# Chthi/Ofighters

Measured on AMD Instinct MI355X. Metric: arena-steps/sec (env.step+obs+policy fwd) at 4096 arenas, 1/2/4/8 MI355X, higher is better.
Workload: dtype f32; 1 GPU; 4096 arenas x 8 ships per GPU, random-bot actions + step + 2D obs rasterise (u8 maps) + bi-head policy forward for 8 ship(s)/arena, trunk shared per arena (BASELINE configs[3]); arenas_per_gpu=4096, ships=8, laser_cap=512, episode_ticks=200, parallelism=arena-sharded x1, RCCL all-reduce of episodic scores only, laser_overflow=0, last_episode_score_sum=70993, last_episode_arenas=4096

## Files before the change

ofighters_amd/csrc/ofx_head.hip:

```cpp
#include "ofx_head.h"
#include "ofx_lowp.h"
#include "ofx_diag.h"
#include <stdlib.h>


typedef float f32x4 __attribute__((ext_vector_type(4)));
typedef float f32x2 __attribute__((ext_vector_type(2)));
#define HD_PS 400
constexpr int HC4_ZERO = 800;
constexpr int HC4_COL = 816, HC4_CPITCH = 416;
constexpr int HC4_STRIDE = HC4_COL + 2 * HC4_CPITCH + 16;
__device__ __forceinline__ int hc4_at(int ln, int t) { return ln < 2 ? ln * 400 + t : HC4_COL + (ln - 2) * HC4_CPITCH + t; }
__device__ __forceinline__ int hc4_pad(int k) { return k < 16 ? HC4_ZERO + k : k < 32 ? HC4_COL + 400 + k - 16 : HC4_COL + HC4_CPITCH + 400 + k - 32; }

__device__ __forceinline__ void hc4_zero_block(const HeadParams2 &p, int tid, int threads) {
  if (blockIdx.x == 0)
    for (int e = tid; e < HC4_STRIDE; e += threads) p.c4[(size_t)p.S * HC4_STRIDE + e] = 0.f;
}

__device__ __forceinline__ float hd_max_raw(float x, float floor) {
  float pinf;
  asm("s_mov_b32 %0, 0x7f800000" : "=s"(pinf));
  return __builtin_amdgcn_fmed3f(x, floor, pinf);
}
// ... 125 lines not shown
    if (t >= 0 && t < 200) {
      int fa, fb, ta, tb; float wf, wt;
      hf_taps(f, 100, fa, fb, wf, p.legacy);
      hf_taps(t, 100, ta, tb, wt, p.legacy);
      const int ba = fa < 2 ? fa : fa - 96, bb = fb < 2 ? fb : fb - 96;
      const float *src = isc ? u2cb : u2rb;
      const float a = src[(ba * 100 + ta) * 4 + ci], bq = src[(ba * 100 + tb) * 4 + ci];
      const float d = src[(bb * 100 + ta) * 4 + ci], g = src[(bb * 100 + tb) * 4 + ci];
      if (!isc) {
        const float top = a + (bq - a) * wt, bot = d + (g - d) * wt;
        v = top + (bot - top) * wf;
      } else {
        const float top = a + (d - a) * wf, bot = bq + (g - bq) * wf;
        v = top + (bot - top) * wt;
      }
    }
    (isc ? U2c : U2r)[(b * 4 + ci) * 202 + t + 1] = v;
  }
  __syncthreads();

  for (int e = tid; e < 4 * 200 * 8; e += HF_THREADS) {
    const int co = e % 8, t = (e / 8) % 200, ln = e / 1600, isc = ln >> 1;
    const int f = (ln & 1) ? 199 : 0;
    float acc = p.b3[co];
#pragma unroll
    for (int d0 = 0; d0 < 3; d0++) {
      const int u = f + d0 - 1;
      if (u < 0 || u > 199) continue;
      const int ub = u < 2 ? u : u - 196;
#pragma unroll
      for (int d1 = 0; d1 < 3; d1++)
#pragma unroll
        for (int ci = 0; ci < 4; ci++) {
          const int dy = isc ? d1 : d0, dx = isc ? d0 : d1;
          const float uv = (isc ? U2c : U2r)[(ub * 4 + ci) * 202 + t + d1];
          acc += p.w3raw[((dy * 3 + dx) * 4 + ci) * 8 + co] * uv;
        }
    }
    u3l[(ln * 200 + t) * 8 + co] = fmaxf(acc, 0.f);
  }
  __syncthreads();
  if (tid < 32) {
    const int co = tid & 7, c = tid >> 3;
    const int rl = (c & 1) ? 1 : 0, x = (c & 2) ? 199 : 0;
    const int cl = (c & 2) ? 3 : 2, y = (c & 1) ? 199 : 0;
    u3l[(cl * 200 + y) * 8 + co] = u3l[(rl * 200 + x) * 8 + co];
  }
  __syncthreads();
  for (int e = tid; e < 4 * 200 * 9; e += HF_THREADS) {
    const int tp = e % 9, cell = e / 9;
    float acc = 0.f;
    for (int ci = 0; ci < 8; ci++) acc = fmaf(p.w4raw[tp * 8 + ci], u3l[cell * 8 + ci], acc);
    p.vfr[(size_t)s * 7200 + e] = acc;
  }

  for (int e = tid; e < 4 * 400; e += HF_THREADS) {
    const int ln = e / 400, t = e - ln * 400, isc = ln >> 1, side = ln & 1;
    float acc = 0.f;
    if (!isc || (t > 0 && t < 399)) {
      const int d0 = side ? 2 : 0;
#pragma unroll
      for (int d1 = 0; d1 < 3; d1++)
#pragma unroll
        for (int ci = 0; ci < 8; ci++) {
          const int tap = isc ? d1 * 3 + d0 : d0 * 3 + d1;
          acc += p.w4raw[tap * 8 + ci] * hf_up(u3l + ln * 1600 + ci, 8, 200, t + d1 - 1, p.legacy);
        }
      if (!isc && (t == 0 || t == 399)) {
        const int cl = t ? 3 : 2, dx = t ? 2 : 0;
        for (int dy = 0; dy < 3; dy++) {
          if (dy == d0) continue;
          const int yy = (side ? 399 : 0) + dy - 1;
          if (yy < 0 || yy > 399) continue;
          for (int ci = 0; ci < 8; ci++) acc += p.w4raw[(dy * 3 + dx) * 8 + ci] * hf_up(u3l + cl * 1600 + ci, 8, 200, yy, p.legacy);
        }
      }
    }
    p.c4[(size_t)s * HC4_STRIDE + hc4_at(ln, t)] = acc;
  }
  if (tid < 64) p.c4[(size_t)s * HC4_STRIDE + hc4_pad(tid)] = 0.f;
}

constexpr int HG_THREADS = 256;
constexpr int HG_L1 = 0;
constexpr int HG_U3 = 0;
constexpr int HG_RB = 6400;
constexpr int HG_CB = HG_RB + 4 * 102 * 4;
constexpr int HG_TOTAL = HG_CB + 4 * 102 * 4;
static_assert(2 * 52 * 52 <= 6400, "l1p fits under u3l");

template <int CIN, int COUT>
__device__ __forceinline__ void hg_corner_w(const float *w, int yc, int xc, int co, float (&wr)[4 * CIN]) {
  const int dy0 = yc == 0 ? 1 : 0, dx0 = xc == 0 ? 1 : 0;
#pragma unroll
  for (int t = 0; t < 4; t++)
#pragma unroll
    for (int ci = 0; ci < CIN; ci++) wr[t * CIN + ci] = w[(((dy0 + (t >> 1)) * 3 + dx0 + (t & 1)) * CIN + ci) * COUT + co];
}
template <int CIN, class G>
__device__ __forceinline__ float hg_corner(G get, int n, int yc, int xc, const float (&wr)[4 * CIN], float bias, int legacy) {
  float acc = bias;
  const int dy0 = yc == 0 ? 1 : 0, dx0 = xc == 0 ? 1 : 0;
#pragma unroll
  for (int a2 = 0; a2 < 2; a2++) {
    int ya, yb; float wy;
    hf_taps(yc + dy0 + a2 - 1, n, ya, yb, wy, legacy);
#pragma unroll
    for (int b2 = 0; b2 < 2; b2++) {
      int xa, xb; float wx;
      hf_taps(xc + dx0 + b2 - 1, n, xa, xb, wx, legacy);
#pragma unroll
      for (int ci = 0; ci < CIN; ci++) {
        const float a = get(ya, xa, ci), b = get(ya, xb, ci), d = get(yb, xa, ci), g = get(yb, xb, ci);
        const float top = a + (b - a) * wx, bot = d + (g - d) * wx;
        acc += wr[(a2 * 2 + b2) * CIN + ci] * (top + (bot - top) * wy);
      }
    }
  }
  return fmaxf(acc, 0.f);
}

constexpr int HG_NB = 6 * 52 + 46 * 6, HG_NE = 2 * HG_NB, HG_PER = (HG_NE + HG_THREADS - 1) / HG_THREADS;
struct alignas(16) HgStage { unsigned v[HG_PER * HG_THREADS]; };
constexpr HgStage hg_make_stage() {
  HgStage t{};
  for (int e0 = 0; e0 < HG_PER * HG_THREADS; e0++) {
    const int e = e0 < HG_NE ? e0 : HG_NE - 1;
    const int ci = e / HG_NB, k = e - ci * HG_NB;
    int r = 0, c = 0;
    if (k < 6 * 52) { const int rr = k / 52; r = rr < 3 ? rr : rr + 46; c = k - rr * 52; }
    else { const int k2 = k - 6 * 52, cc = k2 % 6; r = 3 + k2 / 6; c = cc < 3 ? cc : cc + 46; }
    const int rs = r - 1 < 0 ? 0 : r - 1 > 49 ? 49 : r - 1, cs = c - 1 < 0 ? 0 : c - 1 > 49 ? 49 : c - 1;
    t.v[e0] = (unsigned)((ci * 52 + r) * 52 + c) | (unsigned)((ci * 50 + rs) * 50 + cs) << 16;
  }
  return t;
}
__constant__ HgStage kHgStage = hg_make_stage();

__global__ __launch_bounds__(HG_THREADS) void k_head_frames(HeadParams2 p) {
  __shared__ __align__(16) float sm[HG_TOTAL];
  __shared__ float efr_s[192], w4s[72];
  const int s = hd_ship(p, (int)((blockIdx.x & ~7u) | ((blockIdx.x + (blockIdx.x >> 3)) & 7u)));
  const int tid = threadIdx.x, lane = tid & 63;
  hc4_zero_block(p, tid, HG_THREADS);
  if (s < 0) return;
  const int wv = __builtin_amdgcn_readfirstlane(tid >> 6);
  const int n16 = lane & 15, kq = lane >> 4;
  float *l1p = sm + HG_L1, *u2rb = sm + HG_RB, *u2cb = sm + HG_CB, *u3l = sm + HG_U3;

  constexpr int NE = HG_NE, PER = HG_PER;
  unsigned at[PER];
#pragma unroll
  for (int u = 0; u < PER; u++) at[u] = kHgStage.v[u * HG_THREADS + tid];
  const float efr_v = p.efr[min(tid, 191)], w4_v = p.w4raw[min(tid, 71)];
  float bw2[5];
#pragma unroll
  for (int jj = 0; jj < 5; jj++) bw2[jj] = p.w2fr[(wv * 20 + 4 * jj + kq) * 16 + n16];
  float bw3[9];
#pragma unroll
  for (int jj = 0; jj < 9; jj++) bw3[jj] = p.w3fr[(wv * 36 + 4 * jj + kq) * 16 + n16];
  const float b2v = p.b2[n16 & 3], b3v = p.b3[n16 & 7];
  float wc2[8], wc3[16];
  if (wv == 0) {
    hg_corner_w<2, 4>(p.w2raw, (lane >> 5) ? 99 : 0, ((lane >> 4) & 1) ? 99 : 0, lane & 3, wc2);
    hg_corner_w<4, 8>(p.w3raw, ((lane >> 3) & 1) ? 199 : 0, ((lane >> 3) & 2) ? 199 : 0, lane & 7, wc3);
  }
  {
    float v[PER];
    const float *src = p.up1 + (size_t)s * 5000;
#pragma unroll
    for (int u = 0; u < PER; u++) v[u] = src[at[u] >> 16];
#pragma unroll
    for (int u = 0; u < PER; u++)
      if (u * HG_THREADS + tid < NE) l1p[at[u] & 0xFFFFu] = v[u];
  }
  if (tid < 192) efr_s[tid] = efr_v;
  if (tid < 72) w4s[tid] = w4_v;
  __syncthreads();

#pragma unroll 1
  for (int m = 0; m < 4; m++) {
    const int v = wv;
    const int pp = min(16 * m + n16, 49);
    const int i = v == 0 ? 0 : v == 1 ? 49 : pp, j = v == 2 ? 0 : v == 3 ? 49 : pp;
    const float bias = b2v;
    f32x4 d = {bias, bias, bias, bias};
#pragma unroll
    for (int jj = 0; jj < 5; jj++) {
      const int tap = min(2 * jj + (kq >> 1), 8);
      const float a = l1p[((kq & 1) * 52 + i + tap / 3) * 52 + j + tap % 3];
      d = __builtin_amdgcn_mfma_f32_16x16x4f32(a, bw2[jj], d, 0, 0, 0);
    }
    const int co = n16 & 3, pa = n16 >> 3, pb = (n16 >> 2) & 1;
#pragma unroll
    for (int r = 0; r < 4; r++) {
      const int q = 16 * m + 4 * kq + r;
      if (q >= 50) continue;
      const float val = fmaxf(d[r], 0.f);
      if (v < 2) {
        u2rb[((2 * v + pa) * 102 + 2 * q + pb + 1) * 4 + co] = val;
      } else {
        u2cb[((2 * (v - 2) + pb) * 102 + 2 * q + pa + 1) * 4 + co] = val;
      }
    }
  }
  __syncthreads();
  if (tid < 64) {
    const int co = tid & 3, cx = (tid >> 2) & 1, cy = (tid >> 3) & 1, bx = (tid >> 4) & 1, by = tid >> 5;
    const int y = by ? 98 + cy : cy, x = bx ? 98 + cx : cx;
    const int rb = by ? 2 + cy : cy, cb = bx ? 2 + cx : cx;
    const bool fy = y == 0 || y == 99, fx = x == 0 || x == 99;
    float val;
    if (fy && fx) {
      auto get = [&](int yy, int xx, int ci) { return l1p[(ci * 52 + yy + 1) * 52 + xx + 1]; };
      val = hg_corner<2>(get, 50, y, x, wc2, b2v, p.legacy);
    } else if (fx) {
      val = u2cb[(cb * 102 + y + 1) * 4 + co];
    } else {
      val = u2rb[(rb * 102 + x + 1) * 4 + co];
    }
    if (fy && fx) { u2rb[(rb * 102 + x + 1) * 4 + co] = val; u2cb[(cb * 102 + y + 1) * 4 + co] = val; }
    else if (fx) u2rb[(rb * 102 + x + 1) * 4 + co] = val;
    else u2cb[(cb * 102 + y + 1) * 4 + co] = val;
  }
  __syncthreads();
  if (tid < 128) {
    const int co = tid & 3, b = (tid >> 2) & 3, hi = (tid >> 4) & 1, isc = tid >> 5;
    if (isc < 2) {
      float *ln = (isc ? u2cb : u2rb) + b * 102 * 4;
      ln[(hi ? 101 : 0) * 4 + co] = ln[(hi ? 100 : 1) * 4 + co];
    }
  }
  {
    const float *src = (wv < 2 ? u2rb : u2cb) + ((wv & 1) ? 3 : 0) * 408 + 4;
    float *dst = p.u2fr + (size_t)s * 1600 + wv * 400;
#pragma unroll
    for (int k = 0; k < 7; k++) {
      const int r = lane + 64 * k;
      if (r < 400) dst[r] = src[r];
    }
  }
  __syncthreads();

#pragma unroll 1
  for (int m = 0; m < 7; m++) {
    const int v = wv;
    const int qq = min(16 * m + n16, 99);
    const float *band = (v < 2 ? u2rb : u2cb);
    const int b0 = (v & 1) ? 2 : 0;
    const float bias = b3v;
    f32x4 d = {bias, bias, bias, bias};
#pragma unroll
    for (int jj = 0; jj < 9; jj++) {
      const int ty = jj / 3, tx = jj % 3;
      const int tf = v < 2 ? ty : tx, ta = v < 2 ? tx : ty;
      const int bsel = (v & 1) ? b0 + min(tf, 1) : b0 + max(tf - 1, 0);
      const float a = band[(bsel * 102 + qq + ta) * 4 + kq];
      d = __builtin_amdgcn_mfma_f32_16x16x4f32(a, bw3[jj], d, 0, 0, 0);
    }
    const int co = n16 & 7, par = n16 >> 3;
#pragma unroll
    for (int r = 0; r < 4; r++) {
      const int q = 16 * m + 4 * kq + r;
      if (q < 100) u3l[(v * 200 + 2 * q + par) * 8 + co] = fmaxf(d[r], 0.f);
    }
  }
  __syncthreads();
  if (tid < 32) {
    const int co = tid & 7, c = tid >> 3;
    const int y = (c & 1) ? 199 : 0, x = (c & 2) ? 199 : 0;
    auto get = [&](int yy, int xx, int ci) {
      return u2rb[((yy < 50 ? yy : yy - 96) * 102 + xx + 1) * 4 + ci];
    };
    const float val = hg_corner<4>(get, 100, y, x, wc3, b3v, p.legacy);
    u3l[(((c & 1) ? 1 : 0) * 200 + x) * 8 + co] = val;
    u3l[(((c & 2) ? 3 : 2) * 200 + y) * 8 + co] = val;
  }
  __syncthreads();
  if (tid < 252) {
    const int tp = tid % 9, c0 = tid / 9;
    float wt[8];
#pragma unroll
    for (int ci = 0; ci < 8; ci++) wt[ci] = w4s[tp * 8 + ci];
    float *dst = p.vfr + (size_t)s * 7200 + tid;
    for (int cell = c0; cell < 4 * 200; cell += 28) {
      const f32x4 ua = *reinterpret_cast<const f32x4 *>(u3l + cell * 8), ub = *reinterpret_cast<const f32x4 *>(u3l + cell * 8 + 4);
      float acc = 0.f;
#pragma unroll
      for (int ci = 0; ci < 4; ci++) acc = fmaf(wt[ci], ua[ci], acc);
#pragma unroll
      for (int ci = 0; ci < 4; ci++) acc = fmaf(wt[4 + ci], ub[ci], acc);
      dst[(cell - c0) * 9] = acc;
    }
  }

  {
    const int ln = wv, isc = ln >> 1, side = ln & 1;
    const float *L = u3l + ln * 1600;
    float E[24];
#pragma unroll
    for (int i = 0; i < 24; i++) E[i] = efr_s[(ln * 2 + (lane & 1)) * 24 + i];
    float *dst = p.c4 + (size_t)s * HC4_STRIDE + hc4_at(ln, 0);
#pragma unroll 1
    for (int k = 0; k < 7; k++) {
      const int t = lane + 64 * k, jq = t >> 1;
      float acc = 0.f;
#pragma unroll
      for (int o = 0; o < 3; o++) {
        const float *Lp = L + min(max(jq + o - 1, 0), 199) * 8;
        const f32x4 la = *reinterpret_cast<const f32x4 *>(Lp), lb = *reinterpret_cast<const f32x4 *>(Lp + 4);
#pragma unroll
        for (int ci = 0; ci < 4; ci++) acc += E[o * 8 + ci] * la[ci];
#pragma unroll
        for (int ci = 0; ci < 4; ci++) acc += E[o * 8 + 4 + ci] * lb[ci];
      }
      if (isc && (t == 0 || t == 399)) acc = 0.f;
      if (!isc && (t == 0 || t == 399)) {
        const int cs = t ? 1 : 0;
        const int yq = side ? 199 : 0, a = side ? 1 : 0;
        const float *E2 = efr_s + ((2 + cs) * 2 + a) * 24;
        const float *L2 = u3l + (2 + cs) * 1600;
        for (int o = 0; o < 3; o++) {
          const float *Lp = L2 + min(max(yq + o - 1, 0), 199) * 8;
          for (int ci = 0; ci < 8; ci++) acc += E2[o * 8 + ci] * Lp[ci];
        }
        const int tap = (side ? 2 : 0) * 3 + (cs ? 2 : 0);
        const float *Lc = L + (t ? 199 : 0) * 8;
        for (int ci = 0; ci < 8; ci++) acc -= w4s[tap * 8 + ci] * Lc[ci];
      }
      if (t < 400) dst[t] = acc;
    }
  }
  if (tid < 64) p.c4[(size_t)s * HC4_STRIDE + hc4_pad(tid)] = 0.f;
}

constexpr int HS_GPR = 13;
constexpr int HS_NTILES = 325;
constexpr int HS_NS = 42;
constexpr int HS_NR3 = 16, HS_P3 = 106;
constexpr int HS_PL3 = HS_NR3 * HS_P3 + 4;
constexpr int HS_NV = 9;
constexpr int HS_NR2 = 16, HS_P2 = 56;
constexpr int HS_PL2 = (HS_NR2 + 2) * HS_P2;
static_assert(HS_PL2 % 32 == 16, "uprelu2 plane stride");
constexpr int HS_TABP = 16 * HS_GPR;
static_assert(HS_TABP == 4 * 52, "table period in tiles");
static_assert(4 * (HS_NV * HS_PL3 + 4 * HS_PL2 + HS_TABP + 400) <= 80 * 1024, "two workgroups per CU");
struct alignas(16) HsPick { signed char v[HS_NS][4]; };
constexpr int hs_pairs_done_c(int s) { return s + 2 + ((s + 2) >> 2) < 50 ? s + 2 + ((s + 2) >> 2) : 50; }
constexpr HsPick hs_make_pick() {
  HsPick t{};
  for (int st = 0; st < HS_NS; st++)
    for (int cw = 0; cw < 4; cw++) {
      const int lo = 2 * hs_pairs_done_c(st), hi = 2 * hs_pairs_done_c(st + 1);
      const int at = lo + ((cw - lo) & 3);
      t.v[st][cw] = (signed char)(at < hi ? at >> 1 : -1);
    }
  return t;
}
__constant__ HsPick kHsPick = hs_make_pick();

__device__ __forceinline__ int hs_tiles_done(int s) {
  return s < 0 ? 0 : min(HS_NTILES, 8 * (s + 1) + ((s + 1) >> 3));
}

typedef const volatile __attribute__((address_space(3))) f32x2 hs_lds_v2;

__device__ __forceinline__ void hs_u2_store(float *u2r, int ch, int row, int col, float v) {
  const int slot = (row + 1) & (HS_NR2 - 1);
  float *q = &u2r[ch * HS_PL2 + slot * HS_P2 + col];
  q[0] = v;
  if (slot < 2) q[HS_NR2 * HS_P2] = v;
}

constexpr bool HS_NZ[2][3][3] = {{{1, 1, 0}, {1, 1, 0}, {0, 1, 1}}, {{1, 1, 0}, {0, 1, 1}, {0, 1, 1}}};
constexpr float HS_CH[2][3][3] = {{{0.75f, 0.25f, 0.f}, {0.25f, 0.75f, 0.f}, {0.f, 0.75f, 0.25f}},
                                  {{0.25f, 0.75f, 0.f}, {0.f, 0.75f, 0.25f}, {0.f, 0.25f, 0.75f}}};
constexpr float HS_CL[2][3][3] = {{{0.5f, 0.5f, 0.f}, {0.f, 1.f, 0.f}, {0.f, 0.5f, 0.5f}},
                                  {{0.f, 1.f, 0.f}, {0.f, 0.5f, 0.5f}, {0.f, 0.f, 1.f}}};
static_assert(HS_CH[0][0][0] == HS_CH[0][2][1] && HS_CH[0][0][1] == HS_CH[0][2][2] && HS_CH[1][0][0] == HS_CH[1][2][1] &&
              HS_CH[1][0][1] == HS_CH[1][2][2] && HS_CL[0][0][0] == HS_CL[0][2][1] && HS_CL[0][0][1] == HS_CL[0][2][2] &&
              HS_CL[1][0][0] == HS_CL[1][2][1] && HS_CL[1][0][1] == HS_CL[1][2][2], "the stencil shares the sums of the outer taps");
constexpr int HS_NKT = 7;
constexpr int HS_KT[HS_NKT][2] = {{0, 0}, {0, 1}, {1, 0}, {1, 1}, {1, 2}, {2, 1}, {2, 2}};
__device__ __forceinline__ f32x2 hs_fma2(float c, f32x2 v, f32x2 z) { return __builtin_elementwise_fma((f32x2){c, c}, v, z); }

// ... 533 lines not shown
```

ofighters_amd/csrc/ofx_policy.hip:

```cpp
#include <string.h>

#include "ofx_internal.h"
#include "ofx_blob.h"
#include "ofx_trunk.h"
#include "ofx_head.h"

typedef float f32x16 __attribute__((ext_vector_type(16)));
typedef float f32x4 __attribute__((ext_vector_type(4)));


extern "C" int ofx_policy_layout(const ofx_handle *h, ofx_policy_desc *desc) {
  (void)h;
  if (!desc) { ofx_set_error("ofx_policy_layout: null desc"); return OFX_ERR_INVALID; }
  memset(desc, 0, sizeof(*desc));
  desc->n_tensors = policy_layout(desc->offset, desc->count);
  desc->n_floats = desc->offset[desc->n_tensors];
  return OFX_OK;
}

struct PrepLayout {
  int tw[4], tb[4];
  int uw[3], ub[3];
  int w3mf;
  int w2mf;
// ... 334 lines not shown
    }
    if (u == NB0) {
#pragma unroll
      for (int i = NB0 + NB1; i < NU; i++) a[i] = *reinterpret_cast<const f32x4 *>(ap + 4 * i);
    }
    if ((u & 1) == 0) b4[u >> 1] = *reinterpret_cast<const f32x4 *>(bl + (u >> 1) * 2 * 32 * 4);
    acc = __builtin_amdgcn_mfma_f32_32x32x2f32(kh ? a[u][1] : a[u][0], b4[u >> 1][(2 * u) & 3], acc, 0, 0, 0);
    acc = __builtin_amdgcn_mfma_f32_32x32x2f32(kh ? a[u][3] : a[u][2], b4[u >> 1][(2 * u + 1) & 3], acc, 0, 0, 0);
  }
  if (cv) {
    const float bv = bias ? bias[c] : 0.f;
#pragma unroll
    for (int i = 0; i < 16; i++) {
      const int row = m0 + (i & 3) + 8 * (i >> 2) + 4 * kh;
      if (row < M) {
        float v = acc[i] + bv;
        if (relu) v = fmaxf(v, 0.f);
        C[(size_t)(live ? live[1 + row] : row) * ldc + c] = v;
      }
    }
  }
}

constexpr int kSplitKc = 200;
__global__ __launch_bounds__(256) void k_gemm_f32_splitk(const float *A, int lda, const float *B, int ldb, float *P,
                                                         int M, int N, int tiles_n, int groups_m) {
  constexpr int Kc = kSplitKc, KG = Kc / 4, STEPS = Kc / 8;
  __shared__ __align__(16) float bs[KG * 32 * 4];
  const int tid = threadIdx.x, lane = tid & 63, wv = __builtin_amdgcn_readfirstlane(tid >> 6);
  const int nt = blockIdx.x % tiles_n, rest = blockIdx.x / tiles_n, mg = rest % groups_m, chunk = rest / groups_m;
  const int m0 = (mg * 4 + wv) * 32, n0 = nt * 32;
  const int r = m0 + (lane & 31), c = n0 + (lane & 31), kh = lane >> 5;
  const bool rv = r < M, cv = c < N;
  {
    const float *bp = B + (size_t)chunk * Kc * ldb + (n0 + (tid & 31) < N ? n0 + (tid & 31) : 0);
    f32x4 w[(KG + 7) / 8];
#pragma unroll
    for (int i = 0; i < (KG + 7) / 8; i++) {
      const int g = min((tid >> 5) + 8 * i, KG - 1);
#pragma unroll
      for (int j = 0; j < 4; j++) w[i][j] = bp[(size_t)(4 * g + j) * ldb];
    }
#pragma unroll
    for (int i = 0; i < (KG + 7) / 8; i++) {
      const int g = (tid >> 5) + 8 * i;
      if (g < KG) *reinterpret_cast<f32x4 *>(bs + (g * 32 + (tid & 31)) * 4) = w[i];
    }
  }
  const float *ap = A + (size_t)(rv ? r : 0) * lda + (size_t)chunk * Kc + 4 * kh;
  constexpr int NB0 = 9, NB1 = 8;
  f32x4 a[STEPS];
#pragma unroll
  for (int i = 0; i < NB0; i++) a[i] = *reinterpret_cast<const f32x4 *>(ap + 8 * i);
  __syncthreads();
  if (m0 >= M) return;
  f32x16 acc;
#pragma unroll
  for (int i = 0; i < 16; i++) acc[i] = 0.f;
  const float *bl = bs + (kh * 32 + (lane & 31)) * 4;
#pragma unroll
  for (int s = 0; s < STEPS; s++) {
    if (s == 0) {
#pragma unroll
      for (int i = NB0; i < NB0 + NB1; i++) a[i] = *reinterpret_cast<const f32x4 *>(ap + 8 * i);
    }
    if (s == NB0) {
#pragma unroll
      for (int i = NB0 + NB1; i < STEPS; i++) a[i] = *reinterpret_cast<const f32x4 *>(ap + 8 * i);
    }
    const f32x4 b4 = *reinterpret_cast<const f32x4 *>(bl + s * 2 * 32 * 4);
#pragma unroll
    for (int j = 0; j < 4; j++) acc = __builtin_amdgcn_mfma_f32_32x32x2f32(a[s][j], b4[j], acc, 0, 0, 0);
  }
  if (cv) {
    float *out = P + (size_t)chunk * M * N;
#pragma unroll
    for (int i = 0; i < 16; i++) {
      const int row = m0 + (i & 3) + 8 * (i >> 2) + 4 * kh;
      if (row < M) out[(size_t)row * N + c] = acc[i];
    }
  }
}

struct HeadParams {
  int N, M;
  ofx_state st;
  const float *g1;
  int g1_chunks;
  const float *k1, *b1, *k2, *b2, *k3, *b3;
  const int32_t *live;
  const uint8_t *mask;
  const float *vec8;
  float *d1;
  float *act;
  int32_t *iaction;
};

__global__ __launch_bounds__(256) void k_head_dense(HeadParams p) {
  __shared__ float sd1[4][100];
  __shared__ float sd2[4][50];
  const int lane = threadIdx.x & 63, wv = threadIdx.x >> 6;
  const int item = blockIdx.x * 4 + wv, n_items = p.live ? p.live[0] : p.N * p.M;
  if ((int)blockIdx.x * 4 >= n_items) return;
  const bool on = item < n_items;
  const int s = on ? (p.live ? p.live[1 + item] : item) : 0;
  const int a = s / p.M;
  float vec[8];
  if (on) {
    if (p.vec8) {
#pragma unroll
      for (int k = 0; k < 8; k++) vec[k] = p.vec8[(size_t)s * 8 + k];
    } else {
      vec[0] = (float)p.st.reward[s]; vec[1] = 1.f;
      vec[2] = (float)p.st.ship_px[s]; vec[3] = (float)p.st.ship_py[s];
      vec[4] = (float)PS; vec[5] = (float)PS;
      vec[6] = (float)p.st.ship_x[s]; vec[7] = (float)p.st.ship_y[s];
    }
    for (int o = lane; o < 100; o += 64) {
      float acc = 0.f;
#pragma unroll
      for (int k = 0; k < 8; k++) acc += vec[k] * p.k1[k * 100 + o];
      float g = 0.f;
      for (int ch = 0; ch < p.g1_chunks; ch++) g += p.g1[((size_t)ch * p.N + a) * 100 + o];
      acc += g;
      acc += p.b1[o];
      acc = fmaxf(acc, 0.f);
      sd1[wv][o] = acc;
      p.d1[(size_t)s * 100 + o] = acc;
    }
  }
  __syncthreads();
  if (on && lane < 50) {
    float acc = 0.f;
    for (int k = 0; k < 100; k++) acc += sd1[wv][k] * p.k2[k * 50 + lane];
    sd2[wv][lane] = fmaxf(acc + p.b2[lane], 0.f);
  }
  __syncthreads();
  if (on && lane < 2) {
    float acc = 0.f;
    for (int k = 0; k < 50; k++) acc += sd2[wv][k] * p.k3[k * 2 + lane];
    acc += p.b3[lane];
    if (p.act) p.act[(size_t)s * 2 + lane] = acc;
    const float other = __shfl_xor(acc, 1);
    if (lane == 0 && p.iaction) p.iaction[s] = other > acc ? 1 : 0;
  }
}

__device__ inline float unordered_f32(unsigned o) {
  return __uint_as_float((o & 0x80000000u) ? (o & 0x7FFFFFFFu) : ~o);
}

__global__ void k_policy_finish(int S, const uint8_t *mask, const unsigned long long *best, int32_t *ipointer,
                                float *ptr_max) {
  const int s = blockIdx.x * blockDim.x + threadIdx.x;
  if (s >= S || (mask && !mask[s])) return;
  const bool none = best[s] == 0ull;
  const unsigned k = none ? 0u : ~(unsigned)(best[s] & 0xFFFFFFFFull);
  ipointer[2 * s] = (int)(k % PS);
  ipointer[2 * s + 1] = (int)(k / PS);
  if (ptr_max) ptr_max[s] = none ? __builtin_nanf("") : unordered_f32((unsigned)(best[s] >> 32));
}

__global__ void k_policy_actions(int S, const ofx_state st, const int32_t *iaction, const int32_t *ipointer,
                                 const uint8_t *mask, ofx_action *out) {
  const int s = blockIdx.x * blockDim.x + threadIdx.x;
  if (s >= S || (mask && !mask[s])) return;
  ofx_action a;
  a.valid = st.alive[s] ? 1 : 0;
  a.shoot = iaction[s] == 0;
  a.thrust = iaction[s] == 1;
  a.px = ipointer[2 * s];
  a.py = ipointer[2 * s + 1];
  a._pad = 0;
  out[s] = a;
}

struct PolicyWs {
  float *p1, *p2, *p3, *p4, *g1, *d1, *u0, *up1, *u2fr, *vfr, *c4;
  unsigned long long *best;
  int32_t *iaction, *ipointer, *live;
};

static size_t al(size_t b) { return (b + 255) & ~(size_t)255; }
constexpr int kDense1Chunks = 25;

static int policy_workspace(ofx_handle *h, PolicyWs *ws, size_t N, size_t S) {
  size_t f2, f3, f4;
  ofx_head_frame_bytes(S, &f2, &f3, &f4);
  const size_t sz[] = {ofx_trunk_fused(h, N) ? 0 : al(4ull * N * 8 * 200 * 200), al(4ull * N * 8 * 100 * 100), al(4ull * N * 8 * 50 * 50),
                       al(4ull * N * 5000),          al(4ull * N * 100 * kDense1Chunks), al(4ull * S * 100),
                       al(4ull * S * 625),           al(4ull * S * 2 * 50 * 50),   al(f2), al(f3), al(f4),
                       al(8ull * S),                 al(4ull * S),                 al(8ull * S),
                       al(4ull * (S + 1))};
  size_t total = 0;
  for (size_t b : sz) total += b;
  int rc = ofx_ensure_scratch(h, total);
  if (rc) return rc;
  char *base = (char *)h->scratch;
  void **dst[] = {(void **)&ws->p1,   (void **)&ws->p2,   (void **)&ws->p3,      (void **)&ws->p4,      (void **)&ws->g1,
                  (void **)&ws->d1,   (void **)&ws->u0,   (void **)&ws->up1,     (void **)&ws->u2fr,    (void **)&ws->vfr,
                  (void **)&ws->c4,   (void **)&ws->best, (void **)&ws->iaction, (void **)&ws->ipointer,
                  (void **)&ws->live};
  for (size_t i = 0; i < sizeof(sz) / sizeof(sz[0]); i++) { *dst[i] = base; base += sz[i]; }
  return OFX_OK;
}

int ofx_launch_gemm(ofx_handle *h, const float *A, int lda, const float *B, int ldb, const float *bias, float *C, int ldc,
                    int M, int N, int K, int relu, const int32_t *live) {
  const int tiles_m = (M + 31) / 32, tiles_n = (N + 31) / 32, tiles = tiles_m * tiles_n;
  if (K == 100 && lda % 4 == 0 && ((uintptr_t)A & 15) == 0)
    hipLaunchKernelGGL(k_gemm_f32_k100, dim3((unsigned)(((tiles_m + 3) / 4) * tiles_n)), dim3(256), 0, h->stream, A, lda, B, ldb,
                       bias, C, ldc, M, N, relu, live, tiles_n);
  else
    hipLaunchKernelGGL(k_gemm_f32, dim3((tiles + 3) / 4), dim3(256), 0, h->stream, A, lda, B, ldb, bias, C, ldc, M, N, K,
                       relu, live);
  OFX_HIP(hipGetLastError());
  return OFX_OK;
}

static int policy_prepare(ofx_handle *h, const float *weights, float **slot) {
  const PrepLayout L = prep_layout();
  if (!*slot) {
    OFX_HIP(hipMalloc((void **)slot, sizeof(float) * L.total));
    OFX_HIP(hipMemsetAsync(*slot, 0, sizeof(float) * L.total, h->stream));
  }
  int32_t off[64], cnt[64];
  policy_layout(off, cnt);
  PrepParams pp;
  pp.w = weights; pp.prep = *slot;
  for (int i = 0; i < 4; i++) {
    pp.src_k[i] = off[ofx_t_trunk(i)]; pp.src_b[i] = off[ofx_t_trunk(i, OFX_T_BIAS)]; pp.src_g[i] = off[ofx_t_trunk(i, OFX_T_GAMMA)];
    pp.cin[i] = kTrunkCin[i]; pp.cout[i] = 8; pp.dst_w[i] = L.tw[i]; pp.dst_b[i] = L.tb[i];
  }
  for (int i = 0; i < 3; i++) {
    pp.src_k[4 + i] = off[ofx_t_up(i)]; pp.src_b[4 + i] = off[ofx_t_up(i, OFX_T_BIAS)]; pp.src_g[4 + i] = off[ofx_t_up(i, OFX_T_GAMMA)];
    pp.cin[4 + i] = kUpCin[i]; pp.cout[4 + i] = kUpCout[i]; pp.dst_w[4 + i] = L.uw[i]; pp.dst_b[4 + i] = L.ub[i];
  }
  pp.src_k4 = off[OFX_T_OUT2]; pp.src_b4 = off[OFX_T_OUT2 + 1];
  pp.dst_w4raw = L.w4raw; pp.dst_b4 = L.b4; pp.dst_efr = L.efr;
  pp.dst_w4eff_c = L.w4eff_c; pp.dst_w3mf = L.w3mf; pp.dst_w2mf = L.w2mf; pp.dst_w2fr = L.w2fr; pp.dst_w3fr = L.w3fr; pp.dst_lut1 = L.lut1;
  for (int i = 0; i < 3; i++) pp.dst_wbm[i] = L.wbm[i];
  pp.legacy = h->opt_bilinear_legacy;
  pp.phase = 0;
  hipLaunchKernelGGL(k_policy_prepare, dim3(32), dim3(256), 0, h->stream, pp);
  pp.phase = 1;
  hipLaunchKernelGGL(k_policy_prepare, dim3(4), dim3(256), 0, h->stream, pp);
  OFX_HIP(hipGetLastError());
  return OFX_OK;
}

extern "C" int ofx_policy_pin_weights(ofx_handle *h, const float *weights) {
  if (!h) { ofx_set_error("ofx_policy_pin_weights: null handle"); return OFX_ERR_INVALID; }
  OFX_HIP(hipSetDevice(h->cfg.device));
  h->prep_pinned = nullptr;
  if (!weights) return OFX_OK;
  int rc = policy_prepare(h, weights, &h->prep);
  if (rc) return rc;
  h->prep_pinned = weights;
  return OFX_OK;
}

int ofx_policy_weights_updated(ofx_handle *h, const float *weights) {
  if (h->prep_pinned && h->prep_pinned == weights) return policy_prepare(h, weights, &h->prep);
  return OFX_OK;
}

extern "C" int ofx_set_option(ofx_handle *h, int32_t option, int32_t value) {
  if (!h) { ofx_set_error("ofx_set_option: null handle"); return OFX_ERR_INVALID; }
  switch (option) {
    case OFX_OPT_TRUNK_PLAIN: h->opt_trunk_plain = value != 0; return OFX_OK;
    case OFX_OPT_TRUNK_FUSE:
      if (value < 0 || value > 2) { ofx_set_error("ofx_set_option: OFX_OPT_TRUNK_FUSE takes 0 (auto), 1 (always), 2 (never)"); return OFX_ERR_INVALID; }
      h->opt_trunk_fuse = value; return OFX_OK;
    case OFX_OPT_FRAMES_REF: h->opt_frames_ref = value != 0; return OFX_OK;
    case OFX_OPT_TRUNK_SPARSE:
      if (value && !h->trunk_stat) {
        OFX_HIP(hipSetDevice(h->cfg.device));
        OFX_HIP(hipMalloc((void **)&h->trunk_stat, 4 * sizeof(unsigned long long)));
        OFX_HIP(hipMemsetAsync(h->trunk_stat, 0, 4 * sizeof(unsigned long long), h->stream));
      }
      h->opt_trunk_dense = value == 0; h->opt_trunk_count = value != 0; return OFX_OK;
    case OFX_OPT_FIT_PLAIN: h->opt_fit_plain = value != 0; return OFX_OK;
    case OFX_OPT_POLICY_BF16:
      if (value < 0 || value > 2) { ofx_set_error("ofx_set_option: OFX_OPT_POLICY_BF16 takes 0 (fp32), 1 (bf16 operands), 2 (fp16 operands)"); return OFX_ERR_INVALID; }
      h->opt_policy_lowp = value; return OFX_OK;
    case OFX_OPT_BILINEAR_LEGACY:
      if (h->opt_bilinear_legacy == (value != 0)) return OFX_OK;
      h->opt_bilinear_legacy = value != 0;
      OFX_HIP(hipSetDevice(h->cfg.device));
      return h->prep_pinned ? policy_prepare(h, h->prep_pinned, &h->prep) : OFX_OK;
    default: ofx_set_error("ofx_set_option: unknown option %d", option); return OFX_ERR_INVALID;
  }
}

struct ForwardArgs {
  const float *weights;
  int N, M;
  const unsigned *bits[2];
  size_t bits_stride;
  const float *vec8;
  const uint8_t *ship_mask;
  float *act_values, *heatmap, *ptr_max, *ptr_probe;
  int32_t *iaction, *ipointer;
  const int32_t *probe;
};

static int policy_forward_impl(ofx_handle *h, const ForwardArgs &a) {
  const int N = a.N, S = a.N * a.M;
  const float *weights = a.weights;
  PolicyWs ws;
  int rc = policy_workspace(h, &ws, N, S);
  if (rc) return rc;
  int32_t off[64], cnt[64];
  policy_layout(off, cnt);
  const PrepLayout L = prep_layout();

  const bool pinned = h->prep && h->prep_pinned == weights;
  if (!pinned && (rc = policy_prepare(h, weights, &h->prep_tmp))) return rc;
  const float *prep = pinned ? h->prep : h->prep_tmp;

  const int lowp = a.vec8 == nullptr ? h->opt_policy_lowp : 0;
  TrunkParams tp;
  memset(&tp, 0, sizeof(tp));
  tp.bits[0] = a.bits[0]; tp.bits[1] = a.bits[1]; tp.bits_stride = a.bits_stride; tp.images = N;
  for (int i = 0; i < 4; i++) { tp.tw[i] = prep + L.tw[i]; tp.tb[i] = prep + L.tb[i]; }
  for (int i = 0; i < 3; i++) tp.wbm[i] = prep + L.wbm[i];
  tp.lut1 = prep + L.lut1; tp.zero16 = prep + L.zero16;
  tp.p1 = ws.p1; tp.p2 = ws.p2; tp.p3 = ws.p3; tp.p4 = ws.p4;
  tp.lowp = lowp; tp.sparse = !h->opt_trunk_dense || a.vec8 != nullptr;
  tp.stat = h->opt_trunk_count ? h->trunk_stat : nullptr;
  if ((rc = ofx_launch_trunk(h, tp))) return rc;

  const float *k1 = weights + off[OFX_T_DENSE1];
  {
    static_assert(5000 == kDense1Chunks * kSplitKc, "k_gemm_f32_splitk's chunk");
    const int tiles_n = (100 + 31) / 32, groups_m = ((N + 31) / 32 + 3) / 4;
    hipLaunchKernelGGL(k_gemm_f32_splitk, dim3((unsigned)(tiles_n * groups_m * kDense1Chunks)), dim3(256), 0, h->stream, ws.p4,
                       5000, k1 + 8 * 100, 100, ws.g1, N, 100, tiles_n, groups_m);
    OFX_HIP(hipGetLastError());
  }
  HeadParams hp;
  hp.N = N; hp.M = a.M; hp.st = h->st; hp.vec8 = a.vec8; hp.g1 = ws.g1; hp.g1_chunks = kDense1Chunks;
  hp.k1 = k1; hp.b1 = weights + off[OFX_T_DENSE1 + 1];
  hp.k2 = weights + off[OFX_T_DENSE2]; hp.b2 = weights + off[OFX_T_DENSE2 + 1];
  hp.k3 = weights + off[OFX_T_OUT1]; hp.b3 = weights + off[OFX_T_OUT1 + 1];
  const int32_t *live = nullptr;
  if (a.ship_mask) {
    if ((rc = ofx_head_compact(h, S, a.ship_mask, ws.live))) return rc;
    live = ws.live;
  }
  hp.mask = a.ship_mask; hp.live = live; hp.d1 = ws.d1; hp.act = a.act_values; hp.iaction = a.iaction ? a.iaction : ws.iaction;
  hipLaunchKernelGGL(k_head_dense, dim3((S + 3) / 4), dim3(256), 0, h->stream, hp);
  OFX_HIP(hipGetLastError());

  if ((rc = ofx_launch_gemm(h, ws.d1, 100, weights + off[OFX_T_UPDENSE], 625, weights + off[OFX_T_UPDENSE + 1], ws.u0, 625, S, 625, 100, 1, live)))
    return rc;
  ConvParams up;
  memset(&up, 0, sizeof(up));
  up.live = live; up.images = S; up.legacy = h->opt_bilinear_legacy;
  up.in = ws.u0; up.w = prep + L.uw[0]; up.b = prep + L.ub[0]; up.out = ws.up1;
  if (up.legacy) hipLaunchKernelGGL(k_upconv1<true>, dim3((unsigned)(live && S > 4096 ? 4096 : S)), dim3(256), 0, h->stream, up);
  else hipLaunchKernelGGL(k_upconv1<false>, dim3((unsigned)(live && S > 4096 ? 4096 : S)), dim3(256), 0, h->stream, up);
  OFX_HIP(hipGetLastError());
  OFX_HIP(hipMemsetAsync(ws.best, 0, sizeof(unsigned long long) * S, h->stream));
  HeadParams2 hp2;
  memset(&hp2, 0, sizeof(hp2));
  hp2.S = S; hp2.up1 = ws.up1;
  hp2.w2mf = prep + L.w2mf; hp2.b2 = prep + L.ub[1]; hp2.w2raw = prep + L.uw[1];
  hp2.w3mf = prep + L.w3mf; hp2.b3 = prep + L.ub[2]; hp2.w3raw = prep + L.uw[2];
  hp2.w4eff_c = prep + L.w4eff_c; hp2.b4 = prep + L.b4; hp2.w4raw = prep + L.w4raw;
  hp2.w2fr = prep + L.w2fr; hp2.w3fr = prep + L.w3fr; hp2.efr = prep + L.efr;
  hp2.u2fr = ws.u2fr; hp2.vfr = ws.vfr; hp2.c4 = ws.c4;
  hp2.frames_ref = h->opt_frames_ref; hp2.legacy = h->opt_bilinear_legacy;
  hp2.bf16 = lowp;
  hp2.mask = a.ship_mask; hp2.live = ws.live; hp2.live_ready = a.ship_mask != nullptr; hp2.best = ws.best; hp2.heat = a.heatmap;
  hp2.probe = a.probe; hp2.ptr_probe = a.probe ? a.ptr_probe : nullptr;
  const int pb = h->prof_base;
  hp2.event_base = pb;
  if ((rc = ofx_launch_head(h, hp2))) return rc;
  if (pb >= 0) h->prof_base = pb + 3 < OFX_RING_MAX ? pb + 2 : -1;
  hipLaunchKernelGGL(k_policy_finish, dim3((S + 255) / 256), dim3(256), 0, h->stream, S, a.ship_mask, ws.best,
                     a.ipointer ? a.ipointer : ws.ipointer, a.ptr_max);
  OFX_HIP(hipGetLastError());
  return OFX_OK;
}

static int live_forward_check(ofx_handle *h, const float *weights, const char *who) {
  if (!h || !weights) { ofx_set_error("%s: null argument", who); return OFX_ERR_INVALID; }
  if (!h->spawned) { ofx_set_error("You must execute analyse_battleground first."); return OFX_ERR_STATE; }
  const ofx_config &c = h->cfg;
  if (c.width != PS || c.height != PS) {
    ofx_set_error("%s: the pointer_model takes 400x400 maps (got %d x %d)", who, c.width, c.height);
    return OFX_ERR_INVALID;
  }
  return OFX_OK;
}

static int live_forward(ofx_handle *h, ForwardArgs &a) {
  const ofx_config &c = h->cfg;
  int rc = ofx_launch_raster(h, OFX_MAP_BITS_LSB, nullptr, nullptr);
  if (rc) return rc;
  int32_t *ria, *rip;
  if ((rc = ofx_policy_results(h, &ria, &rip))) return rc;
  if (!a.iaction) a.iaction = ria;
  if (!a.ipointer) a.ipointer = rip;
  a.N = c.n_arenas; a.M = c.n_ships;
  a.bits[0] = (const unsigned *)h->maps[OFX_MAP_BITS_LSB][0]; a.bits[1] = (const unsigned *)h->maps[OFX_MAP_BITS_LSB][1];
  a.bits_stride = (size_t)(PS * PS) >> 5;
  return policy_forward_impl(h, a);
}

extern "C" int ofx_policy_forward(ofx_handle *h, const float *weights, const uint8_t *ship_mask, float *act_values,
                                  int32_t *iaction, int32_t *ipointer, float *heatmap) {
  int rc = live_forward_check(h, weights, "ofx_policy_forward");
  if (rc) return rc;
  OFX_HIP(hipSetDevice(h->cfg.device));
  ForwardArgs a{};
  a.weights = weights;
  a.ship_mask = ship_mask; a.act_values = act_values; a.iaction = iaction; a.ipointer = ipointer; a.heatmap = heatmap;
  return live_forward(h, a);
}

static ForwardArgs obs_args(const float *weights, int32_t n_obs, const void *bits, const float *vec8) {
  const size_t words = (size_t)(PS * PS) >> 5;
  ForwardArgs a{};
  a.weights = weights; a.N = n_obs; a.M = 1;
  a.bits[0] = (const unsigned *)bits; a.bits[1] = a.bits[0] + words; a.bits_stride = 2 * words;
  a.vec8 = vec8;
  return a;
}

extern "C" int ofx_policy_forward_obs(ofx_handle *h, const float *weights, int32_t n_obs, const void *bits,
                                      const float *vec8, float *act_values, int32_t *iaction, int32_t *ipointer,
                                      float *ptr_max, const int32_t *probe, float *ptr_probe) {
  if (!h || !weights || !bits || !vec8 || n_obs < 1) { ofx_set_error("ofx_policy_forward_obs: bad argument"); return OFX_ERR_INVALID; }
// ... 197 lines not shown
```

Baseline: 232,300 arena-steps/s.

## Batch 8 ships per dense-head block with shared weights; unroll head_frames loops

k_head_dense now processes 8 ships per 256-thread block. It stages k1/k2/k3 and the biases in LDS and reduces the split-K g1 partials once per arena instead of once per ship, and the dense2 layer computes two ships per thread. This cuts repeated global weight reads and the redundant chunk reductions for ships that share an arena's trunk output. Separately, k_head_frames gets a 4-wave occupancy launch bound, fully unrolled conv loops with precomputed band pointers, and a row/column template specialisation, at some risk of higher register pressure or spills.

Measured after the change: 233,800 arena-steps/s, median of 6. About the same (+0.6%).

```diff
diff --git a/ofighters_amd/csrc/ofx_head.hip b/ofighters_amd/csrc/ofx_head.hip
--- a/ofighters_amd/csrc/ofx_head.hip
+++ b/ofighters_amd/csrc/ofx_head.hip
@@ -231,6 +231,7 @@
 }
 
 constexpr int HG_THREADS = 256;
+template <bool B> struct HgBool { static constexpr bool value = B; };
 constexpr int HG_L1 = 0;
 constexpr int HG_U3 = 0;
 constexpr int HG_RB = 6400;
@@ -286,7 +287,7 @@
 }
 __constant__ HgStage kHgStage = hg_make_stage();
 
-__global__ __launch_bounds__(HG_THREADS) void k_head_frames(HeadParams2 p) {
+__global__ __launch_bounds__(HG_THREADS, 4) void k_head_frames(HeadParams2 p) {
   __shared__ __align__(16) float sm[HG_TOTAL];
   __shared__ float efr_s[192], w4s[72];
   const int s = hd_ship(p, (int)((blockIdx.x & ~7u) | ((blockIdx.x + (blockIdx.x >> 3)) & 7u)));
@@ -327,7 +328,7 @@
   if (tid < 72) w4s[tid] = w4_v;
   __syncthreads();
 
-#pragma unroll 1
+#pragma unroll
   for (int m = 0; m < 4; m++) {
     const int v = wv;
     const int pp = min(16 * m + n16, 49);
@@ -391,29 +392,38 @@
   }
   __syncthreads();
 
-#pragma unroll 1
-  for (int m = 0; m < 7; m++) {
+  auto lines = [&](auto row_lines) {
+    constexpr bool ROW = decltype(row_lines)::value;
     const int v = wv;
-    const int qq = min(16 * m + n16, 99);
-    const float *band = (v < 2 ? u2rb : u2cb);
+    const float *band = ROW ? u2rb : u2cb;
     const int b0 = (v & 1) ? 2 : 0;
-    const float bias = b3v;
-    f32x4 d = {bias, bias, bias, bias};
-#pragma unroll
-    for (int jj = 0; jj < 9; jj++) {
-      const int ty = jj / 3, tx = jj % 3;
-      const int tf = v < 2 ? ty : tx, ta = v < 2 ? tx : ty;
+    const float *bp[3], *bp6[3];
+#pragma unroll
+    for (int tf = 0; tf < 3; tf++) {
       const int bsel = (v & 1) ? b0 + min(tf, 1) : b0 + max(tf - 1, 0);
-      const float a = band[(bsel * 102 + qq + ta) * 4 + kq];
-      d = __builtin_amdgcn_mfma_f32_16x16x4f32(a, bw3[jj], d, 0, 0, 0);
+      bp[tf] = band + (bsel * 102 + n16) * 4 + kq;
+      bp6[tf] = band + (bsel * 102 + min(96 + n16, 99)) * 4 + kq;
     }
     const int co = n16 & 7, par = n16 >> 3;
-#pragma unroll
-    for (int r = 0; r < 4; r++) {
-      const int q = 16 * m + 4 * kq + r;
-      if (q < 100) u3l[(v * 200 + 2 * q + par) * 8 + co] = fmaxf(d[r], 0.f);
-    }
-  }
+    float *up = u3l + (v * 200 + 8 * kq + par) * 8 + co;
+#pragma unroll
+    for (int m = 0; m < 7; m++) {
+      const float bias = b3v;
+      f32x4 d = {bias, bias, bias, bias};
+#pragma unroll
+      for (int jj = 0; jj < 9; jj++) {
+        const int ty = jj / 3, tx = jj % 3;
+        const int tf = ROW ? ty : tx, ta = ROW ? tx : ty;
+        const float a = m < 6 ? bp[tf][(16 * m + ta) * 4] : bp6[tf][ta * 4];
+        d = __builtin_amdgcn_mfma_f32_16x16x4f32(a, bw3[jj], d, 0, 0, 0);
+      }
+#pragma unroll
+      for (int r = 0; r < 4; r++)
+        if (m < 6 || kq == 0) up[(32 * m + 2 * r) * 8] = fmaxf(d[r], 0.f);
+    }
+  };
+  if (wv < 2) lines(HgBool<true>{});
+  else lines(HgBool<false>{});
   __syncthreads();
   if (tid < 32) {
     const int co = tid & 7, c = tid >> 3;
@@ -432,7 +442,7 @@
 #pragma unroll
     for (int ci = 0; ci < 8; ci++) wt[ci] = w4s[tp * 8 + ci];
     float *dst = p.vfr + (size_t)s * 7200 + tid;
-    for (int cell = c0; cell < 4 * 200; cell += 28) {
+    auto plane = [&](int cell) {
       const f32x4 ua = *reinterpret_cast<const f32x4 *>(u3l + cell * 8), ub = *reinterpret_cast<const f32x4 *>(u3l + cell * 8 + 4);
       float acc = 0.f;
 #pragma unroll
@@ -440,7 +450,14 @@
 #pragma unroll
       for (int ci = 0; ci < 4; ci++) acc = fmaf(wt[4 + ci], ub[ci], acc);
       dst[(cell - c0) * 9] = acc;
-    }
+    };
+    static_assert(28 * 28 + 16 == 4 * 200, "vfr passes");
+#pragma unroll 1
+    for (int i0 = 0; i0 < 28; i0 += 7) {
+#pragma unroll
+      for (int i = 0; i < 7; i++) plane(c0 + 28 * (i0 + i));
+    }
+    if (c0 < 16) plane(c0 + 28 * 28);
   }
 
   {
@@ -450,7 +467,7 @@
 #pragma unroll
     for (int i = 0; i < 24; i++) E[i] = efr_s[(ln * 2 + (lane & 1)) * 24 + i];
     float *dst = p.c4 + (size_t)s * HC4_STRIDE + hc4_at(ln, 0);
-#pragma unroll 1
+#pragma unroll
     for (int k = 0; k < 7; k++) {
       const int t = lane + 64 * k, jq = t >> 1;
       float acc = 0.f;
diff --git a/ofighters_amd/csrc/ofx_policy.hip b/ofighters_amd/csrc/ofx_policy.hip
--- a/ofighters_amd/csrc/ofx_policy.hip
+++ b/ofighters_amd/csrc/ofx_policy.hip
@@ -440,11 +440,12 @@
   }
 }
 
+constexpr int kDense1Chunks = 25;
+constexpr int kDenseShips = 8;
 struct HeadParams {
   int N, M;
   ofx_state st;
   const float *g1;
-  int g1_chunks;
   const float *k1, *b1, *k2, *b2, *k3, *b3;
   const int32_t *live;
   const uint8_t *mask;
@@ -455,52 +456,112 @@
 };
 
 __global__ __launch_bounds__(256) void k_head_dense(HeadParams p) {
-  __shared__ float sd1[4][100];
-  __shared__ float sd2[4][50];
-  const int lane = threadIdx.x & 63, wv = threadIdx.x >> 6;
-  const int item = blockIdx.x * 4 + wv, n_items = p.live ? p.live[0] : p.N * p.M;
-  if ((int)blockIdx.x * 4 >= n_items) return;
-  const bool on = item < n_items;
-  const int s = on ? (p.live ? p.live[1 + item] : item) : 0;
-  const int a = s / p.M;
-  float vec[8];
-  if (on) {
-    if (p.vec8) {
-#pragma unroll
-      for (int k = 0; k < 8; k++) vec[k] = p.vec8[(size_t)s * 8 + k];
-    } else {
-      vec[0] = (float)p.st.reward[s]; vec[1] = 1.f;
-      vec[2] = (float)p.st.ship_px[s]; vec[3] = (float)p.st.ship_py[s];
-      vec[4] = (float)PS; vec[5] = (float)PS;
-      vec[6] = (float)p.st.ship_x[s]; vec[7] = (float)p.st.ship_y[s];
-    }
-    for (int o = lane; o < 100; o += 64) {
+  constexpr int G = kDenseShips, NK2 = (100 * 50 + 255) / 256, NK1 = (8 * 100 + 255) / 256, NR = (G * 100 + 255) / 256;
+  __shared__ __align__(16) float sk2[100 * 50];
+  __shared__ __align__(16) float sd1[G][100];
+  __shared__ float sk1[8 * 100], sb1[100], sb2[50], sk3[50 * 2], sb3[2];
+  __shared__ float sg[G][100], sd2[G][50], sv[G][8];
+  __shared__ int s_ship[G], s_lead[G];
+  const int tid = threadIdx.x;
+  float rk2[NK2], rk1[NK1];
+#pragma unroll
+  for (int i = 0; i < NK2; i++) rk2[i] = p.k2[min(tid + 256 * i, 100 * 50 - 1)];
+#pragma unroll
+  for (int i = 0; i < NK1; i++) rk1[i] = p.k1[min(tid + 256 * i, 8 * 100 - 1)];
+  const float rb1 = p.b1[min(tid, 99)], rk3 = p.k3[min(tid, 99)], rb2 = p.b2[min(tid, 49)], rb3 = p.b3[min(tid, 1)];
+  const int item0 = blockIdx.x * G, n_items = p.live ? p.live[0] : p.N * p.M;
+  if (item0 >= n_items) return;
+  if (tid < 64) {
+    const int slot = tid >> 3, k = tid & 7, item = item0 + slot;
+    const bool on = item < n_items;
+    const int s = on ? (p.live ? p.live[1 + item] : item) : 0;
+    float v;
+    if (p.vec8) v = p.vec8[(size_t)s * 8 + k];
+    else if (k == 1) v = 1.f;
+    else if (k == 4 || k == 5) v = (float)PS;
+    else v = (float)(k == 0 ? p.st.reward : k == 2 ? p.st.ship_px : k == 3 ? p.st.ship_py : k == 6 ? p.st.ship_x : p.st.ship_y)[s];
+    sv[slot][k] = v;
+    const int t = tid & (G - 1), it = item0 + t;
+    const bool ton = it < n_items;
+    const int ts = ton ? (p.live ? p.live[1 + it] : it) : 0;
+    const int ta = ton ? ts / p.M : -1 - t;
+    const int prev = __shfl_up(ta, 1);
+    const unsigned long long heads = __ballot(tid < G && (t == 0 || prev != ta));
+    if (tid < G) {
+      s_ship[t] = ton ? ts : -1;
+      s_lead[t] = 31 - __clz((unsigned)heads & ((2u << t) - 1u));
+    }
+  }
+#pragma unroll
+  for (int i = 0; i < NR; i++) {
+    const int idx = tid + 256 * i, slot = idx / 100, o = idx - slot * 100, item = item0 + slot;
+    if (idx < G * 100 && item < n_items) {
+      const int a = (p.live ? p.live[1 + item] : item) / p.M;
+      const int ap = slot == 0 ? -1 : (p.live ? p.live[item] : item - 1) / p.M;
+      if (a != ap) {
+        float part[kDense1Chunks];
+#pragma unroll
+        for (int ch = 0; ch < kDense1Chunks; ch++) part[ch] = p.g1[((size_t)ch * p.N + a) * 100 + o];
+        float g = 0.f;
+#pragma unroll
+        for (int ch = 0; ch < kDense1Chunks; ch++) g += part[ch];
+        sg[slot][o] = g;
+      }
+    }
+  }
+#pragma unroll
+  for (int i = 0; i < NK2; i++)
+    if (tid + 256 * i < 100 * 50) sk2[tid + 256 * i] = rk2[i];
+#pragma unroll
+  for (int i = 0; i < NK1; i++)
+    if (tid + 256 * i < 8 * 100) sk1[tid + 256 * i] = rk1[i];
+  if (tid < 100) { sb1[tid] = rb1; sk3[tid] = rk3; }
+  if (tid < 50) sb2[tid] = rb2;
+  if (tid < 2) sb3[tid] = rb3;
+  __syncthreads();
+#pragma unroll
+  for (int i = 0; i < NR; i++) {
+    const int idx = tid + 256 * i, slot = min(idx / 100, G - 1), o = idx - (idx / 100) * 100, s = s_ship[slot];
+    if (idx < G * 100 && s >= 0) {
       float acc = 0.f;
 #pragma unroll
-      for (int k = 0; k < 8; k++) acc += vec[k] * p.k1[k * 100 + o];
-      float g = 0.f;
-      for (int ch = 0; ch < p.g1_chunks; ch++) g += p.g1[((size_t)ch * p.N + a) * 100 + o];
+      for (int k = 0; k < 8; k++) acc += sv[slot][k] * sk1[k * 100 + o];
+      const float g = sg[s_lead[slot]][o];
       acc += g;
-      acc += p.b1[o];
+      acc += sb1[o];
       acc = fmaxf(acc, 0.f);
-      sd1[wv][o] = acc;
+      sd1[slot][o] = acc;
       p.d1[(size_t)s * 100 + o] = acc;
     }
   }
   __syncthreads();
-  if (on && lane < 50) {
+  if (tid < 200) {
+    const int q = tid / 50, o = tid - q * 50;
+    float acc0 = 0.f, acc1 = 0.f;
+#pragma unroll 5
+    for (int k = 0; k < 100; k += 4) {
+      const f32x4 x0 = *reinterpret_cast<const f32x4 *>(&sd1[q][k]), x1 = *reinterpret_cast<const f32x4 *>(&sd1[q + 4][k]);
+#pragma unroll
+      for (int j = 0; j < 4; j++) {
+        const float w = sk2[(k + j) * 50 + o];
+        acc0 += x0[j] * w;
+        acc1 += x1[j] * w;
+      }
+    }
+    sd2[q][o] = fmaxf(acc0 + sb2[o], 0.f);
+    sd2[q + 4][o] = fmaxf(acc1 + sb2[o], 0.f);
+  }
+  __syncthreads();
+  if (tid < 2 * G) {
+    const int slot = tid >> 1, j = tid & 1, s = s_ship[slot];
     float acc = 0.f;
-    for (int k = 0; k < 100; k++) acc += sd1[wv][k] * p.k2[k * 50 + lane];
-    sd2[wv][lane] = fmaxf(acc + p.b2[lane], 0.f);
-  }
-  __syncthreads();
-  if (on && lane < 2) {
-    float acc = 0.f;
-    for (int k = 0; k < 50; k++) acc += sd2[wv][k] * p.k3[k * 2 + lane];
-    acc += p.b3[lane];
-    if (p.act) p.act[(size_t)s * 2 + lane] = acc;
+    for (int k = 0; k < 50; k++) acc += sd2[slot][k] * sk3[k * 2 + j];
+    acc += sb3[j];
     const float other = __shfl_xor(acc, 1);
-    if (lane == 0 && p.iaction) p.iaction[s] = other > acc ? 1 : 0;
+    if (s >= 0) {
+      if (p.act) p.act[(size_t)s * 2 + j] = acc;
+      if (j == 0 && p.iaction) p.iaction[s] = other > acc ? 1 : 0;
+    }
   }
 }
 
@@ -540,8 +601,6 @@
 };
 
 static size_t al(size_t b) { return (b + 255) & ~(size_t)255; }
-constexpr int kDense1Chunks = 25;
-
 static int policy_workspace(ofx_handle *h, PolicyWs *ws, size_t N, size_t S) {
   size_t f2, f3, f4;
   ofx_head_frame_bytes(S, &f2, &f3, &f4);
@@ -698,7 +757,7 @@
     OFX_HIP(hipGetLastError());
   }
   HeadParams hp;
-  hp.N = N; hp.M = a.M; hp.st = h->st; hp.vec8 = a.vec8; hp.g1 = ws.g1; hp.g1_chunks = kDense1Chunks;
+  hp.N = N; hp.M = a.M; hp.st = h->st; hp.vec8 = a.vec8; hp.g1 = ws.g1;
   hp.k1 = k1; hp.b1 = weights + off[OFX_T_DENSE1 + 1];
   hp.k2 = weights + off[OFX_T_DENSE2]; hp.b2 = weights + off[OFX_T_DENSE2 + 1];
   hp.k3 = weights + off[OFX_T_OUT1]; hp.b3 = weights + off[OFX_T_OUT1 + 1];
@@ -708,7 +767,7 @@
     live = ws.live;
   }
   hp.mask = a.ship_mask; hp.live = live; hp.d1 = ws.d1; hp.act = a.act_values; hp.iaction = a.iaction ? a.iaction : ws.iaction;
-  hipLaunchKernelGGL(k_head_dense, dim3((S + 3) / 4), dim3(256), 0, h->stream, hp);
+  hipLaunchKernelGGL(k_head_dense, dim3((S + kDenseShips - 1) / kDenseShips), dim3(256), 0, h->stream, hp);
   OFX_HIP(hipGetLastError());
 
   if ((rc = ofx_launch_gemm(h, ws.d1, 100, weights + off[OFX_T_UPDENSE], 625, weights + off[OFX_T_UPDENSE + 1], ws.u0, 625, S, 625, 100, 1, live)))
```
